# tooHotSpot/FGN

Measured on AMD Instinct MI355X. Metric: query-imgs/sec (3-way 3-shot, 800x1333 FGN simple_test), higher is better.
Workload: dtype f32; 1 GPU; cfg3: COCO2VOC 3-way 3-shot, query 3x800x1333, supports 9x3x256^2, ResNet-50-C4, R<=300 proposals, D<=100 detections, 1 episode(s) per GPU per step; h2d_in_step=True, gt_mask_rle_in_step=True, world_size_seen=1, phase_lock=rpn, caller_streams=2, support_cache=False, hip_graph=True, winograd_3x3=F(4x4,3x3)

## Files before the change

fgn_amd/csrc/conv_igemm.hip:

```cpp
#include "common.h"
#include <cstdlib>

struct ConvParams {
    const float* x = nullptr;
    const float* w = nullptr;
    float* y = nullptr;
    const float* scale = nullptr;
    const float* shift = nullptr;
    const float* residual = nullptr;
    const float* in_scale = nullptr;
    const int32_t* n_img_dev = nullptr;
    int n_img = 0, H = 1, W = 1, Cin = 0, Ho = 1, Wo = 1, Cout = 0, KH = 1, KW = 1, stride = 1, pad = 0;
    int a_img_div = 1;
    int relu = 0;
    int K = 0;
    int n_tiles_n = 0;
    int band_nt = 0, band_mt = 0;
    float* ws = nullptr;
    int splits = 1, kt_per_split = 0;
#ifdef FGN_EXPERIMENTS
    int32_t* tickets = nullptr;
    int32_t* sched = nullptr;
    int sk_U = 0, sk_dp = 0;
#endif
// ... 1160 lines not shown
        p.x = xs[i]; p.w = w_packed; p.y = ys[i]; p.scale = scale; p.shift = shift;
        p.n_img = ns[i]; p.H = Hs[i]; p.W = Ws[i]; p.Cin = Cin; p.Cout = Cout; p.KH = KH; p.KW = KW;
        p.stride = stride; p.pad = pad; p.relu = relu;
        p.Ho = g.Ho; p.Wo = g.Wo; p.K = g.K; p.x_bytes = g.x_bytes; p.w_bytes = g.w_bytes;
        p.kt_per_split = p.K / BK;
        p.n_tiles_n = cdiv(Cout, 64);
        const int m_tiles = cdiv((int)g.M, 64);
        set_band(p, 64, m_tiles, 64ll * p.K * 4);
        tiles[i] = (m_tiles * p.n_tiles_n + 7) / 8 * 8;
    }
    constexpr int NST = CONV_DMA_STAGES;
    const size_t dlds = std::max((size_t)NST * (64 + 64) * BK, (size_t)64 * (64 + 4)) * sizeof(float);
    const dim3 grid(tiles[0] + tiles[1]), wg(256);
    return Cin != 4 ? launch_kernel<conv_igemm_dma_pair_kernel<64, 64, 32, 32, NST, 4, 0>>(grid, wg, dlds, stream, ps[0], ps[1], tiles[0])
                    : launch_kernel<conv_igemm_dma_pair_kernel<64, 64, 32, 32, NST, 4, 2>>(grid, wg, dlds, stream, ps[0], ps[1], tiles[0]);
}

static int x3_pick_bm(long long M, int Cout, int K, int grp_rows, int grp_valid, int bm) {
    if (bm == 64 || bm == 128) return (grp_rows && grp_rows % bm) ? 0 : bm;
    if (grp_rows && grp_rows % 64) return 0;
    const int nt = cdiv(Cout, X3_BN);
    if (Cout * 10 < nt * X3_BN * 7) return 0;
    if (((M + 63) / 64) * nt < 192) return 0;
    const long long groups = grp_rows ? M / grp_rows : 1;
    const long long valid = grp_rows ? std::min<long long>(grp_valid > 0 ? grp_valid : grp_rows, grp_rows) : M;
    const long long rows64 = (valid + 63) / 64 * 64, rows128 = (valid + 127) / 128 * 128;
    if (K >= 256 && (!grp_rows || grp_rows % 128 == 0) && rows128 * 100 <= rows64 * 108 && groups * (rows128 / 128) * nt >= 400)
        return 128;
    return 64;
}

template <int WMW, int RB, int NT, int NST, bool SH16>
static int launch_x3_cfg(ConvParams& p, int M_max, hipStream_t stream) {
    constexpr int BM = 32 * RB * WMW;
    const int m_tiles = cdiv(M_max, BM);
    set_band(p, BM, m_tiles, (long long)X3_BN * p.K * 6);
    const int tiles = m_tiles * p.n_tiles_n;
    static unsigned long long ok = 0ull;
    hipError_t attr = fgn_allow_full_lds(reinterpret_cast<const void*>(conv_pw_x3_kernel<WMW, RB, NT, NST, SH16>), &ok);
    if (attr != hipSuccess) return (int)attr;
    const size_t lds = (size_t)NST * (BM * 128 + X3_B_STAGE);
    const int per_cu = (int)(160 * 1024 / lds);
    const int grid = std::min(256 * per_cu, (tiles + 7) / 8 * 8);
    p.stamp = fgn_next_stamp_record();
    FGN_LAUNCH_TIMED((conv_pw_x3_kernel<WMW, RB, NT, NST, SH16>), dim3(grid), dim3(128 * WMW), lds, stream, p, tiles);
    FGN_LAUNCH_CHECK();
    return FGN_OK;
}

static int launch_x3(const ConvParams& p0, int M_max, int bm, int nterms, hipStream_t stream) {
    ConvParams p = p0;
    if (!p.w3 || p.npad3 % X3_BN || p.npad3 < p.Cout || (p.Cout & 3) || p.K % BK || p.K < 2 * BK || p.splits != 1) return FGN_ERR_SHAPE;
    p.n_tiles_n = cdiv(p.Cout, X3_BN);
#ifdef FGN_EXPERIMENTS
    if (bm >= 2000) {
        const int b = bm - 2000;
        if (x3_pick_bm(M_max, p.Cout, p.K, p.grp_rows, p.grp_valid, b == 129 ? 128 : b) == 0) return FGN_ERR_SHAPE;
        if (b == 129) return nterms == 9 ? launch_x3_cfg<4, 1, 9, 3, false>(p, M_max, stream) : launch_x3_cfg<4, 1, 6, 3, false>(p, M_max, stream);
        if (b == 128) return launch_x3_cfg<2, 2, 6, 2, false>(p, M_max, stream);
        if (b == 64) return nterms == 9 ? launch_x3_cfg<2, 1, 9, 2, false>(p, M_max, stream) : launch_x3_cfg<2, 1, 6, 2, false>(p, M_max, stream);
        return FGN_ERR_SHAPE;
    }
#endif
    if (bm != 0 && bm != 64 && bm != 128) return FGN_ERR_SHAPE;
    const int BM = x3_pick_bm(M_max, p.Cout, p.K, p.grp_rows, p.grp_valid, bm);
    if (BM == 0) return FGN_ERR_SHAPE;
    if (nterms == 9) return BM == 64 ? launch_x3_cfg<2, 1, 9, 2, true>(p, M_max, stream) : FGN_ERR_SHAPE;
    return BM == 128 ? launch_x3_cfg<2, 2, 6, 2, true>(p, M_max, stream) : launch_x3_cfg<2, 1, 6, 2, true>(p, M_max, stream);
}

extern "C" size_t fgn_x3_image_bytes(int K, int npad, int n_groups) { return (size_t)n_groups * K * npad * 6; }
extern "C" int fgn_x3_row_tile(long long M, int Cout, int K, int grp_rows, int grp_valid) {
    return x3_pick_bm(M, Cout, K, grp_rows, grp_valid, 0);
}

#if defined(X3_PHASES) || defined(H2_PHASES)
static unsigned long long* g_x3_ph = nullptr;
extern "C" int fgn_x3_phases(unsigned long long* host16) {
    if (!g_x3_ph) return FGN_ERR_ARG;
    if (hipDeviceSynchronize() != hipSuccess) return FGN_ERR_ARG;
    if (hipMemcpy(host16, g_x3_ph, 128, hipMemcpyDeviceToHost) != hipSuccess) return FGN_ERR_ARG;
    return hipMemset(g_x3_ph, 0, 128) == hipSuccess ? FGN_OK : FGN_ERR_ARG;
}
#endif

static int h2_pick(long long M, int Cout, int K, int grp_rows, int grp_valid, int bm) {
    if (bm == 264) return (grp_rows && grp_rows % 128) ? 0 : 264;
    if (bm != 0) return x3_pick_bm(M, Cout, K, grp_rows, grp_valid, bm);
    if (Cout <= 64) {
        if (grp_rows && grp_rows % 128) return 0;
        if (Cout < 48 || (M + 127) / 128 < 256) return 0;
        return 264;
    }
    const int bm_x3 = x3_pick_bm(M, Cout, K, grp_rows, grp_valid, 0);
    return (bm_x3 == 128 && !grp_rows) ? 64 : bm_x3;
}

template <int WMW, int WNW, int RB, int NST, bool IM2COL, int KG = 1>
static int launch_h2_cfg(ConvParams& p, const H2Im2col& q2, int M_max, hipStream_t stream) {
    constexpr int BM = 32 * RB * WMW, BN = 64 * WNW;
    const int m_tiles = cdiv(M_max, BM);
    p.n_tiles_n = cdiv(p.Cout, BN);
    set_band(p, BM, m_tiles, (long long)BN * p.K * 4);
    const int tiles = m_tiles * p.n_tiles_n;
    static unsigned long long ok = 0ull;
    hipError_t attr = fgn_allow_full_lds(reinterpret_cast<const void*>(conv_pw_h2_kernel<WMW, WNW, RB, NST, IM2COL, KG>), &ok);
    if (attr != hipSuccess) return (int)attr;
    const size_t lds = (size_t)KG * NST * (BM * 128 + 2 * BN * 64);
    const int per_cu = std::min(3, (int)(160 * 1024 / lds));
    const int grid = std::min(256 * per_cu, (tiles + 7) / 8 * 8);
    p.stamp = fgn_next_stamp_record();
    FGN_LAUNCH_TIMED((conv_pw_h2_kernel<WMW, WNW, RB, NST, IM2COL, KG>), dim3(grid), dim3(64 * WMW * WNW * KG), lds, stream, p, q2, tiles);
    FGN_LAUNCH_CHECK();
    return FGN_OK;
}

extern "C" size_t fgn_h2_image_bytes(int K, int npad, int n_groups) { return (size_t)n_groups * npad * ((size_t)K * 4 + 4); }
extern "C" int fgn_h2_row_tile(long long M, int Cout, int K, int grp_rows, int grp_valid) {
    return h2_pick(M, Cout, K, grp_rows, grp_valid, 0);
}

constexpr int H2_KG_MIN_KTILES = 8;
constexpr int H2_BM_KG2 = 1064;
extern "C" int fgn_h2_k_groups(long long M, int Cout, int K, int grp_rows, int grp_valid) {
    if (h2_pick(M, Cout, K, grp_rows, grp_valid, 0) != 64 || grp_rows != 0 || K % BK) return 1;
    const int kt = K / BK;
    if ((kt & 1) || kt < H2_KG_MIN_KTILES) return 1;
    return cdiv(M, 64) * (long long)cdiv(Cout, H2_BN) <= 256 ? 2 : 1;
}

static int launch_h2(const ConvParams& p0, int M_max, int n_groups, int bm, hipStream_t stream, const H2Im2col* im = nullptr) {
    ConvParams p = p0;
    if (!p.w3 || p.npad3 % H2_BN || p.npad3 < p.Cout || (p.Cout & 3) || p.K % BK || p.K < 2 * BK || p.splits != 1) return FGN_ERR_SHAPE;
    const size_t img = (size_t)n_groups * p.K * p.npad3 * 4;
    p.w3_bytes = (unsigned)img;
    p.w_inv = reinterpret_cast<const float*>(static_cast<const char*>(p.w3) + img);
    H2Im2col none;
    none.y1 = nullptr; none.x_off0 = none.x_off1 = 0u; none.M0 = none.M1 = 0; none.H1 = none.W1 = none.Ho1 = none.Wo1 = 1; none.cin_shift = 0;
    if (bm != 0 && bm != 64 && bm != 128 && bm != 264 && bm != H2_BM_KG2) return FGN_ERR_SHAPE;
    if (bm == H2_BM_KG2 && ((p.K / BK) % 2 || p.K / BK < 4)) return FGN_ERR_SHAPE;
    const int cfg = h2_pick(M_max, p.Cout, p.K, p.grp_rows, p.grp_valid, bm == H2_BM_KG2 ? 64 : bm);
    if (cfg == 0) return FGN_ERR_SHAPE;
    const int kgroups = bm == H2_BM_KG2 ? 2 : (bm == 0 ? fgn_h2_k_groups(M_max, p.Cout, p.K, p.grp_rows, p.grp_valid) : 1);
    if (kgroups == 2)
        return im ? launch_h2_cfg<2, 2, 1, 2, true, 2>(p, *im, M_max, stream) : launch_h2_cfg<2, 2, 1, 2, false, 2>(p, none, M_max, stream);
    if (im) {
        if (cfg == 264) return launch_h2_cfg<4, 1, 1, 2, true>(p, *im, M_max, stream);
        return cfg == 128 ? launch_h2_cfg<2, 2, 2, 2, true>(p, *im, M_max, stream) : launch_h2_cfg<2, 2, 1, 2, true>(p, *im, M_max, stream);
    }
    if (cfg == 264) return launch_h2_cfg<4, 1, 1, 2, false>(p, none, M_max, stream);
    return cfg == 128 ? launch_h2_cfg<2, 2, 2, 2, false>(p, none, M_max, stream) : launch_h2_cfg<2, 2, 1, 2, false>(p, none, M_max, stream);
}

extern "C" int fgn_conv2d_pair_h2_bm_nhwc_f32(const float* x0, int n_img0, int H0, int W0, const float* x1, int n_img1, int H1,
                                              int W1, const void* w_h2, float* y0, float* y1, const float* scale,
                                              const float* shift, int Cin, int Cout, int cout_pad, int KH, int KW, int stride,
                                              int pad, int relu, int bm, hipStream_t stream) {
    if (!x0 || !w_h2 || !y0 || (x1 && !y1)) return FGN_ERR_ARG;
    if (n_img0 <= 0 || (x1 && n_img1 <= 0)) return FGN_ERR_SHAPE;
    const int ct = Cin / BK;
    if (Cin % BK || (ct & (ct - 1)) || KH != KW || (KW != 1 && KW != 3) || stride < 1 || pad < 0 || (Cout & 3) ||
        cout_pad % H2_BN || cout_pad < Cout || H0 <= 0 || W0 <= 0)
        return FGN_ERR_SHAPE;
    const int Ho0 = (H0 + 2 * pad - KH) / stride + 1, Wo0 = (W0 + 2 * pad - KW) / stride + 1;
    const int Ho1 = x1 ? (H1 + 2 * pad - KH) / stride + 1 : 1, Wo1 = x1 ? (W1 + 2 * pad - KW) / stride + 1 : 1;
    if (Ho0 <= 0 || Wo0 <= 0 || Ho1 <= 0 || Wo1 <= 0) return FGN_ERR_SHAPE;
// ... 71 lines not shown
}

extern "C" int fgn_conv1x1_h2_nhwc_f32(const float* x, const void* w_h2, float* y, const float* scale, const float* shift,
                                       const float* residual, const int32_t* n_img_dev, int n_img, int H, int W, int Cin,
                                       int Cout, int cout_pad, int relu, hipStream_t stream) {
    ConvParams p;
    const int rc = describe_conv1x1(p, MATH_H2, x, w_h2, y, scale, shift, residual, n_img_dev, n_img, H, W, Cin, Cout, cout_pad, relu);
    if (rc != FGN_DESCRIBED) return rc;
    return launch_h2(p, n_img * H * W, 1, 0, stream);
}

static int describe_dual(ConvParams& p, const GemmMath& m, const float* x, const float* x2, const int32_t* x2_rows,
                         int x2_total_rows, const void* w, float* y, const float* shift, int rows, int Cin1, int Cin2,
                         int Cout, int cout_pad, int relu) {
    if (!x || !x2 || !w || !y) return FGN_ERR_ARG;
    if (rows <= 0) return FGN_OK;
    if (Cin1 % BK || Cin2 % BK || Cin1 <= 0 || Cin2 <= 0 || (Cout & 3) || cout_pad % m.bn || cout_pad < Cout) return FGN_ERR_SHAPE;
    if ((!x2_rows && x2_total_rows != rows) || x2_total_rows < 1) return FGN_ERR_ARG;
    const long long K = (long long)Cin1 + Cin2;
    const long long xb = (long long)rows * Cin1 * 4, x2b = (long long)x2_total_rows * Cin2 * 4;
    const long long wb = gemm_weight_bytes(m, K, cout_pad, 1);
    if (xb >= 0x7fffff00ll || x2b >= 0x7fffff00ll || wb >= 0x7fffff00ll || (long long)rows * Cout >= (1ll << 31)) return FGN_ERR_SHAPE;
    p.x = x; p.y = y; p.shift = shift;
    p.x2 = x2; p.x2_bytes = (unsigned)x2b; p.kt1 = Cin1 / BK; p.cin2 = Cin2; p.x2_rows = x2_rows;
    p.n_img = rows; p.Cin = Cin1; p.Cout = Cout; p.relu = relu; p.K = (int)K;
    p.kt_per_split = (int)K / BK; p.x_bytes = (unsigned)xb;
    gemm_set_weights(p, m, w, wb, cout_pad);
    return FGN_DESCRIBED;
}

extern "C" int fgn_conv1x1_dual_nhwc_f32(const float* x, const float* x2, const int32_t* x2_rows, int x2_total_rows,
                                         const float* w_packed, float* y, const float* shift, int rows, int Cin1, int Cin2,
                                         int Cout, int cout_pad, int relu, hipStream_t stream) {
    ConvParams p;
    const int rc = describe_dual(p, MATH_F32, x, x2, x2_rows, x2_total_rows, w_packed, y, shift, rows, Cin1, Cin2, Cout, cout_pad, relu);
    if (rc != FGN_DESCRIBED) return rc;
    p.n_tiles_n = cdiv(Cout, 64);
    const int m_tiles = cdiv(rows, 64);
    set_band(p, 64, m_tiles, 64ll * p.K * 4);
    return launch_persist(p, m_tiles * p.n_tiles_n, stream);
}

extern "C" int fgn_conv1x1_dual_x3_nhwc_f32(const float* x, const float* x2, const int32_t* x2_rows, int x2_total_rows,
                                            const void* w_x3, float* y, const float* shift, int rows, int Cin1, int Cin2,
                                            int Cout, int cout_pad, int relu, hipStream_t stream) {
    ConvParams p;
    const int rc = describe_dual(p, MATH_X3, x, x2, x2_rows, x2_total_rows, w_x3, y, shift, rows, Cin1, Cin2, Cout, cout_pad, relu);
    if (rc != FGN_DESCRIBED) return rc;
    return launch_x3(p, rows, 0, 6, stream);
}

extern "C" int fgn_conv1x1_dual_h2_nhwc_f32(const float* x, const float* x2, const int32_t* x2_rows, int x2_total_rows,
                                            const void* w_h2, float* y, const float* shift, int rows, int Cin1, int Cin2,
                                            int Cout, int cout_pad, int relu, hipStream_t stream) {
    ConvParams p;
    const int rc = describe_dual(p, MATH_H2, x, x2, x2_rows, x2_total_rows, w_h2, y, shift, rows, Cin1, Cin2, Cout, cout_pad, relu);
    if (rc != FGN_DESCRIBED) return rc;
    return launch_h2(p, rows, 1, 0, stream);
}

static int describe_gemm(ConvParams& p, const GemmMath& m, const float* x, const void* w, float* y, const float* shift,
                         const float* residual, int rows, int K, int Cout, int npad, int relu, int grp_rows, int grp_valid,
                         int n_groups) {
    if (!x || !w || !y) return FGN_ERR_ARG;
    if (rows <= 0) return FGN_OK;
    if (K % BK || K <= 0 || (Cout & 3) || npad % m.bn || npad < Cout || n_groups < 1) return FGN_ERR_SHAPE;
    if (n_groups > 1 && (grp_rows <= 0 || (long long)n_groups * grp_rows != rows || grp_valid > grp_rows)) return FGN_ERR_SHAPE;
    const long long xb = (long long)rows * K * 4, wb = gemm_weight_bytes(m, K, npad, n_groups);
    if (xb >= 0x7fffff00ll || wb >= 0x7fffff00ll || (long long)rows * Cout >= (1ll << 31)) return FGN_ERR_SHAPE;
    p.x = x; p.y = y; p.shift = shift; p.residual = residual;
    p.n_img = rows; p.Cin = K; p.Cout = Cout; p.relu = relu; p.K = K; p.kt_per_split = K / BK; p.x_bytes = (unsigned)xb;
    p.grp_rows = n_groups > 1 ? grp_rows : 0; p.grp_valid = grp_valid;
    gemm_set_weights(p, m, w, wb, npad);
    return FGN_DESCRIBED;
}

extern "C" int fgn_gemm_x3_f32(const float* x, const void* w3, float* y, const float* shift, const float* residual,
                               int rows, int K, int Cout, int npad, int relu, int grp_rows, int grp_valid, int n_groups,
                               int bm, int nterms, hipStream_t stream) {
    ConvParams p;
    const int rc = describe_gemm(p, MATH_X3, x, w3, y, shift, residual, rows, K, Cout, npad, relu, grp_rows, grp_valid, n_groups);
    if (rc != FGN_DESCRIBED) return rc;
#ifdef X3_PHASES
    if (!g_x3_ph && (hipMalloc(&g_x3_ph, 128) != hipSuccess || hipMemset(g_x3_ph, 0, 128) != hipSuccess)) return FGN_ERR_ARG;
    p.ws = reinterpret_cast<float*>(g_x3_ph);
#endif
    return launch_x3(p, rows, bm, nterms, stream);
}

extern "C" int fgn_gemm_h2_f32(const float* x, const void* w_h2, float* y, const float* shift, const float* residual,
                               int rows, int K, int Cout, int npad, int relu, int grp_rows, int grp_valid, int n_groups,
                               int bm, hipStream_t stream) {
    ConvParams p;
    const int rc = describe_gemm(p, MATH_H2, x, w_h2, y, shift, residual, rows, K, Cout, npad, relu, grp_rows, grp_valid, n_groups);
    if (rc != FGN_DESCRIBED) return rc;
#ifdef H2_PHASES
    if (!g_x3_ph && (hipMalloc(&g_x3_ph, 128) != hipSuccess || hipMemset(g_x3_ph, 0, 128) != hipSuccess)) return FGN_ERR_ARG;
    p.ws = reinterpret_cast<float*>(g_x3_ph);
#endif
    return launch_h2(p, rows, n_groups, bm, stream);
}

extern "C" int fgn_winograd_t_pad(int tiles_total) { return (tiles_total + 127) / 128 * 128; }

static int describe_winograd_gemm(ConvParams& p, const GemmMath& m, const float* V, const void* U, float* Mo,
                                  const int32_t* n_img_dev, int n_img, int tiles_per_img, int t_pad, int Cin, int Cout,
                                  int cout_pad, int n_groups) {
    if (!V || !U || !Mo) return FGN_ERR_ARG;
    if (n_img <= 0) return FGN_OK;
    if (Cin % BK != 0 || (m.deep && Cin < 2 * BK) || Cout % 4 != 0 || cout_pad % m.bn != 0 || cout_pad < Cout || t_pad % 64 != 0 ||
        (n_groups != 16 && n_groups != 36) || (long long)n_img * tiles_per_img > t_pad)
        return FGN_ERR_SHAPE;
    const long long rows = (long long)n_groups * t_pad;
    const long long xb = rows * Cin * 4, wb = gemm_weight_bytes(m, Cin, cout_pad, n_groups);
    if (xb >= 0x7fffff00ll || wb >= 0x7fffff00ll || rows * Cout >= (1ll << 31)) return FGN_ERR_SHAPE;
    p.x = V; p.y = Mo;
    p.n_img = (int)rows; p.Cin = Cin; p.Cout = Cout; p.K = Cin; p.kt_per_split = Cin / BK; p.x_bytes = (unsigned)xb;
    p.grp_rows = t_pad; p.grp_valid = n_img * tiles_per_img; p.grp_items = n_img;
    p.grp_rows_per_item = tiles_per_img; p.grp_count_dev = n_img_dev;
    gemm_set_weights(p, m, U, wb, cout_pad);
    if (!m.image_bytes) p.grp_w_stride = cout_pad * Cin;
    return FGN_DESCRIBED;
}

extern "C" int fgn_winograd_gemm_f32(const float* V, const float* U, float* Mo, const int32_t* n_img_dev, int n_img,
                                     int tiles_per_img, int t_pad, int Cin, int Cout, int cout_pad, int n_groups,
                                     hipStream_t stream) {
    ConvParams p;
    const int rc = describe_winograd_gemm(p, MATH_F32, V, U, Mo, n_img_dev, n_img, tiles_per_img, t_pad, Cin, Cout, cout_pad, n_groups);
    if (rc != FGN_DESCRIBED) return rc;
#ifdef FGN_EXPERIMENTS
    {
        int rc2 = FGN_OK;
        if (fgn_exp_pointwise(p, p.n_img, 4, true, t_pad, stream, &rc2)) return rc2;
    }
#endif
    return launch_cfg<64, 64, 32, 32, 4>(p, p.n_img, pointwise_mode(4, p.n_img, Cout, 1), stream);
}

extern "C" int fgn_winograd_gemm_x3_f32(const float* V, const void* U_x3, float* Mo, const int32_t* n_img_dev, int n_img,
                                        int tiles_per_img, int t_pad, int Cin, int Cout, int cout_pad, int n_groups,
                                        hipStream_t stream) {
    ConvParams p;
    const int rc = describe_winograd_gemm(p, MATH_X3, V, U_x3, Mo, n_img_dev, n_img, tiles_per_img, t_pad, Cin, Cout, cout_pad, n_groups);
    if (rc != FGN_DESCRIBED) return rc;
    return launch_x3(p, p.n_img, 0, 6, stream);
}

extern "C" int fgn_winograd_gemm_h2_f32(const float* V, const void* U_h2, float* Mo, const int32_t* n_img_dev, int n_img,
                                        int tiles_per_img, int t_pad, int Cin, int Cout, int cout_pad, int n_groups,
                                        hipStream_t stream) {
    ConvParams p;
    const int rc = describe_winograd_gemm(p, MATH_H2, V, U_h2, Mo, n_img_dev, n_img, tiles_per_img, t_pad, Cin, Cout, cout_pad, n_groups);
    if (rc != FGN_DESCRIBED) return rc;
    return launch_h2(p, p.n_img, n_groups, 0, stream);
}
```

fgn_amd/csrc/conv_pw_h2.h:

```cpp
#pragma once

typedef _Float16 f16x8_t __attribute__((ext_vector_type(8)));

struct H2Frag { f16x8_t hi, lo; };

__device__ __forceinline__ void h2_split4(const float x0, const float x1, const float x2, const float x3, const float s,
                                          unsigned& h01, unsigned& h23, unsigned& l01, unsigned& l23) {
    asm("v_fma_mixlo_f16 %0, %4, %8, 0\n\t"
        "v_fma_mixlo_f16 %1, %6, %8, 0\n\t"
        "v_fma_mixhi_f16 %0, %5, %8, 0\n\t"
        "v_fma_mixhi_f16 %1, %7, %8, 0\n\t"
        "v_fma_mixlo_f16 %2, %4, %8, -%0 op_sel:[0,0,0] op_sel_hi:[0,0,1]\n\t"
        "v_fma_mixlo_f16 %3, %6, %8, -%1 op_sel:[0,0,0] op_sel_hi:[0,0,1]\n\t"
        "v_fma_mixhi_f16 %2, %5, %8, -%0 op_sel:[0,0,1] op_sel_hi:[0,0,1]\n\t"
        "v_fma_mixhi_f16 %3, %7, %8, -%1 op_sel:[0,0,1] op_sel_hi:[0,0,1]\n\t"
        "s_nop 1"
        : "=&v"(h01), "=&v"(h23), "=&v"(l01), "=&v"(l23)
        : "v"(x0), "v"(x1), "v"(x2), "v"(x3), "s"(s));
}

__device__ __forceinline__ void h2_split4_step(const int step, const float x0, const float x1, const float x2, const float x3,
                                               const float s, unsigned& h01, unsigned& h23, unsigned& l01, unsigned& l23) {
    if (step == 0)
        asm("v_fma_mixlo_f16 %0, %2, %4, 0\n\t"
            "v_fma_mixlo_f16 %1, %3, %4, 0"
            : "=&v"(h01), "=&v"(h23) : "v"(x0), "v"(x2), "s"(s));
    else if (step == 1)
        asm("v_fma_mixhi_f16 %0, %2, %4, 0\n\t"
            "v_fma_mixhi_f16 %1, %3, %4, 0"
            : "+v"(h01), "+v"(h23) : "v"(x1), "v"(x3), "s"(s));
    else if (step == 2)
        asm("v_fma_mixlo_f16 %0, %2, %4, -%5 op_sel:[0,0,0] op_sel_hi:[0,0,1]\n\t"
            "v_fma_mixlo_f16 %1, %3, %4, -%6 op_sel:[0,0,0] op_sel_hi:[0,0,1]"
            : "=&v"(l01), "=&v"(l23) : "v"(x0), "v"(x2), "s"(s), "v"(h01), "v"(h23));
    else
        asm("v_fma_mixhi_f16 %0, %2, %4, -%5 op_sel:[0,0,1] op_sel_hi:[0,0,1]\n\t"
            "v_fma_mixhi_f16 %1, %3, %4, -%6 op_sel:[0,0,1] op_sel_hi:[0,0,1]"
            : "+v"(l01), "+v"(l23) : "v"(x1), "v"(x3), "s"(s), "v"(h01), "v"(h23));
}

__device__ __forceinline__ H2Frag h2_split(const float4& a, const float4& b, const float s) {
    unsigned h[4], l[4];
    h2_split4(a.x, a.y, a.z, a.w, s, h[0], h[1], l[0], l[1]);
    h2_split4(b.x, b.y, b.z, b.w, s, h[2], h[3], l[2], l[3]);
    H2Frag f;
    f.hi = __builtin_bit_cast(f16x8_t, make_uint4(h[0], h[1], h[2], h[3]));
    f.lo = __builtin_bit_cast(f16x8_t, make_uint4(l[0], l[1], l[2], l[3]));
    return f;
}

__device__ __forceinline__ float h2_absmax16(const float4& a, const float4& b, const float4& c, const float4& d) {
    float m;
    asm("v_max3_f32 %0, |%1|, |%2|, 0\n\t"
        "v_max3_f32 %0, |%3|, |%4|, %0\n\t"
        "v_max3_f32 %0, |%5|, |%6|, %0\n\t"
        "v_max3_f32 %0, |%7|, |%8|, %0\n\t"
        "v_max3_f32 %0, |%9|, |%10|, %0\n\t"
        "v_max3_f32 %0, |%11|, |%12|, %0\n\t"
        "v_max3_f32 %0, |%13|, |%14|, %0\n\t"
        "v_max3_f32 %0, |%15|, |%16|, %0"
        : "=&v"(m)
        : "v"(a.x), "v"(a.y), "v"(a.z), "v"(a.w), "v"(b.x), "v"(b.y), "v"(b.z), "v"(b.w),
          "v"(c.x), "v"(c.y), "v"(c.z), "v"(c.w), "v"(d.x), "v"(d.y), "v"(d.z), "v"(d.w));
    return m;
}

constexpr int H2_BN = 128;

struct H2Im2col {
    float* y1;
    unsigned x_off0, x_off1;
    int M0, M1;
    int H1, W1, Ho1, Wo1;
    int cin_shift;
};

#ifdef H2_PHASES
#define H2_T(i) do { const unsigned long long now_ = __builtin_amdgcn_s_memtime(); ph_[i] += now_ - last_; last_ = now_; } while (0)
#else
#define H2_T(i) do { } while (0)
#endif
template <int WMW, int WNW, int RB, int NST, bool IM2COL, int KG = 1>
__global__ __launch_bounds__(64 * WMW * WNW * KG, KG == 1 ? 2 : 1) void conv_pw_h2_kernel(const ConvParams p, const H2Im2col q2, const int total_tiles) {
    constexpr int BM = 32 * RB * WMW, BN = 64 * WNW, NW = WMW * WNW, NTHR_G = 64 * NW, NTHR = NTHR_G * KG;
    static_assert(KG == 1 || KG == 2, "one or two K-groups");
    constexpr int A_LD = BM / 8 / NW;
    constexpr int A_STAGE = BM * 128;
    constexpr int B_STAGE = 2 * BN * 64;
    constexpr int STAGE = A_STAGE + B_STAGE;
    constexpr int BQ = BN / 16;
    constexpr int B_LD = 2 * BQ / NW;
    static_assert(A_LD * 8 * NW == BM && B_LD * NW == 2 * BQ, "tile / wave split");
    constexpr int PER = A_LD + B_LD;
    constexpr int ROWS_PER_PASS = NTHR_G / 8;
    constexpr bool OLD_CURSOR = KG == 2 && !IM2COL;
    static_assert(NST == 2, "a ring of two stages: one K-tile in flight ahead of the one being multiplied");
    extern __shared__ __attribute__((aligned(16))) unsigned char smem_h2[];

    const int t = threadIdx.x, lane = t & 63;
    const int kg = KG == 1 ? 0 : __builtin_amdgcn_readfirstlane((t >> 6) / NW);
    const int wv = KG == 1 ? t >> 6 : (t >> 6) % NW;
    const int tg = KG == 1 ? t : t % NTHR_G;
    const int wm = wv / WNW, wn = wv % WNW;
    const int M = IM2COL ? q2.M0 + q2.M1 : (p.n_img_dev ? min(p.n_img, *p.n_img_dev) : p.n_img) * p.Ho * p.Wo;
    int grp_valid = p.grp_valid;
    if (p.grp_rows && p.grp_count_dev) grp_valid = min(grp_valid, min(p.grp_items, *p.grp_count_dev) * p.grp_rows_per_item);

    float a_s = 1.f, a_inv = 1.f;

    const int col4 = tg & 7, row0 = tg >> 3;
    const int src_c4 = col4 ^ ((row0 >> 1) & 7);
    const i32x4 x_rs = make_rsrc(p.x, p.x_bytes);
    const i32x4 w_rs = make_rsrc(p.w3, p.w3_bytes);
    const bool dual = !IM2COL && p.x2 != nullptr;
    const i32x4 x2_rs = make_rsrc(dual ? p.x2 : p.x, dual ? p.x2_bytes : p.x_bytes);
    const int KT = p.K / BK / KG;
    const unsigned kt_bytes = (unsigned)(2 * p.npad3 * 64);
    const unsigned lds_base = __builtin_amdgcn_readfirstlane((unsigned)reinterpret_cast<size_t>(smem_h2) + kg * (NST * STAGE));
    const unsigned wave_row_bytes = __builtin_amdgcn_readfirstlane(wv) * 8 * 128;
    constexpr unsigned OOB = 0x7ffffff0u;

    const int nq = total_tiles >> 3, nr = total_tiles & 7;
    auto coords = [&](int tile, int& m0, int& n0) -> bool {
        const int xcd = tile & 7, idx = tile >> 3;
        const int bid = (xcd < nr ? xcd * (nq + 1) : nr * (nq + 1) + (xcd - nr) * nq) + idx;
        int tile_m = bid / p.n_tiles_n;
        int tile_n = bid - tile_m * p.n_tiles_n;
        if (p.band_nt > 0) {
            const int per_grp = p.band_mt * p.n_tiles_n;
            const int grp = bid / per_grp;
            int r = bid - grp * per_grp;
            const int per_band = p.band_mt * p.band_nt;
            const int band = r / per_band;
            r -= band * per_band;
            const int mi = r / p.band_nt;
            tile_m = grp * p.band_mt + mi;
            tile_n = band * p.band_nt + (r - mi * p.band_nt);
        }
        m0 = tile_m * BM;
        n0 = tile_n * BN;
        if (m0 >= M) return false;
        if (p.grp_rows && m0 - (m0 / p.grp_rows) * p.grp_rows >= grp_valid) return false;
        return true;
    };
    auto next_active = [&](int tile, int& m0, int& n0) -> int {
        for (; tile < total_tiles; tile += gridDim.x)
            if (coords(tile, m0, n0)) return tile;
        return -1;
    };

    struct Offs { unsigned a[A_LD], a2[A_LD], b[B_LD]; };
    unsigned b_lds[B_LD];
#pragma unroll
    for (int i = 0; i < B_LD; ++i) {
        const int q = wv + NW * i;
        b_lds[i] = __builtin_amdgcn_readfirstlane((unsigned)(A_STAGE + (q / BQ) * (BN * 64) + (q % BQ) * 1024));
    }
    auto offsets = [&](int m0, int n0) -> Offs {
        Offs o;
        const int g_end = p.grp_rows ? (m0 / p.grp_rows) * p.grp_rows + grp_valid : M;
#pragma unroll
        for (int i = 0; i < A_LD; ++i) {
            const int m = m0 + row0 + ROWS_PER_PASS * i;
            if constexpr (IM2COL) {
                o.a[i] = 0u; o.a2[i] = 0u;
                if (m < M) {
                    const bool t1 = m >= q2.M0;
                    const int mm = t1 ? m - q2.M0 : m;
                    const int H = t1 ? q2.H1 : p.H, W = t1 ? q2.W1 : p.W, Wo = t1 ? q2.Wo1 : p.Wo;
                    const int HoWo = (t1 ? q2.Ho1 : p.Ho) * Wo;
                    const int img = mm / HoWo;
                    const int rem = mm - img * HoWo;
                    const int oy = rem / Wo;
                    const int ox = rem - oy * Wo;
                    const int iy0 = oy * p.stride - p.pad, ix0 = ox * p.stride - p.pad;
                    o.a[i] = (t1 ? q2.x_off1 : q2.x_off0) + (unsigned)((((img * H + iy0) * W + ix0) * p.Cin + src_c4 * 4) * 4);
                    unsigned tm = t1 ? 0x80000000u : 0u;
                    int tp = 0;
// ... 72 lines not shown
            const unsigned voff = ok ? o.a[i] + ((o.a2[i] >> 31) ? c_off1 : c_off0) : OOB;
            lds_dma16_s(x_rs, dst, voff, 0u);
        } else {
            const bool second = c_ko >= ko1;
            i32x4 rs;
            rs[0] = second ? x2_rs[0] : x_rs[0]; rs[1] = second ? x2_rs[1] : x_rs[1];
            rs[2] = second ? x2_rs[2] : x_rs[2]; rs[3] = x_rs[3];
            lds_dma16_s(rs, dst, second ? o.a2[i] : o.a[i], second ? c_ko - ko1 : c_ko);
        }
    };

    auto issue_step = [&](const Offs& o, const int step, const unsigned wr) {
        const int kt = step * KG + kg;
        const unsigned st = lds_base + wr;
        const unsigned sa = st + wave_row_bytes;
        const unsigned ko = (unsigned)(kt * BK * 4);
        if (dual && kt >= p.kt1) {
            const unsigned ko2 = (unsigned)((kt - p.kt1) * BK * 4);
#pragma unroll
            for (int i = 0; i < A_LD; ++i) lds_dma16_s(x2_rs, sa + i * ROWS_PER_PASS * 128, o.a2[i], ko2);
        } else {
#pragma unroll
            for (int i = 0; i < A_LD; ++i) lds_dma16_s(x_rs, sa + i * ROWS_PER_PASS * 128, o.a[i], ko);
        }
        const unsigned kb = (unsigned)kt * kt_bytes;
#pragma unroll
        for (int i = 0; i < B_LD; ++i) lds_dma16_s(w_rs, st + b_lds[i], o.b[i], kb);
    };

    const int r16 = lane & 15, g4 = lane >> 4;
    const int a16_row = wm * 32 * RB + r16;
    const unsigned a16_sw = (unsigned)((a16_row >> 1) & 7);
    const unsigned a16_rd0 = (unsigned)(a16_row * 128) + ((((unsigned)g4) ^ a16_sw) << 4);
    const unsigned a16_rd1 = (unsigned)(a16_row * 128) + ((((unsigned)(g4 + 4)) ^ a16_sw) << 4);
    const int n16 = wn * 64 + r16;
    const unsigned tau16 = (0x1230u >> (4 * ((n16 >> 2) & 3))) & 3u;
    const unsigned b16_rd = (unsigned)(A_STAGE + n16 * 64) + ((((unsigned)g4) ^ tau16) << 4);

    if (p.stamp && t == 0 && blockIdx.x == 0) atomicExch(p.stamp, __builtin_amdgcn_s_memrealtime());
    auto leave = [&]() {
        if (!p.stamp || t != 0) return;
        const unsigned shard = blockIdx.x & 7u;
        const unsigned long long in_shard = (gridDim.x - shard + 7u) / 8u;
        unsigned long long* const sc = p.stamp + 8 * (1 + shard);
        if (atomicAdd(sc, 1ull) != in_shard - 1) return;
        atomicExch(sc, 0ull);
        const unsigned long long shards = gridDim.x < 8u ? gridDim.x : 8u;
        if (atomicAdd(p.stamp + 2, 1ull) != shards - 1) return;
        const unsigned long long d = __builtin_amdgcn_s_memrealtime() - atomicExch(p.stamp, 0ull);
        atomicExch(p.stamp + 2, 0ull);
        atomicAdd(p.stamp + 1, d);
        atomicAdd(p.stamp + 3, 1ull);
        atomicMin(p.stamp + 4, d);
        atomicMax(p.stamp + 5, d);
    };

    int m0, n0, nm0 = 0, nn0 = 0;
    int tile = next_active(blockIdx.x, m0, n0);
    if (tile < 0) { leave(); return; }
    Offs cur = offsets(m0, n0);
    int ntile = next_active(tile + gridDim.x, nm0, nn0);
    auto following = [&]() -> Offs { return ntile >= 0 ? offsets(nm0, nn0) : cur; };
    Offs nxt = following();
    int ic_kt = 0;
    bool ic_next = false;
    auto issue_one = [&](const unsigned wr) {
        if (!ic_next) {
            issue_step(cur, ic_kt, wr);
            if (++ic_kt == KT) { ic_next = true; ic_kt = 0; }
        } else {
            if (ntile < 0 || ic_kt >= KT) return;
            issue_step(nxt, ic_kt, wr);
            ++ic_kt;
        }
    };
    if constexpr (OLD_CURSOR) {
        issue_one(0u);
    } else {
        seek(0);
#pragma unroll
        for (int i = 0; i < PER; ++i) piece(cur, 0u, i);
        advance();
    }
    unsigned rd = 0u;
#ifdef H2_PHASES
    unsigned long long ph_[7] = {0, 0, 0, 0, 0, 0, 0}, last_ = __builtin_amdgcn_s_memtime();
    const unsigned long long begin_ = last_;
#endif

    while (true) {
        f32x4 acc[2 * RB][4];
#pragma unroll
        for (int i = 0; i < 2 * RB; ++i)
#pragma unroll
            for (int j = 0; j < 4; ++j) acc[i][j] = f32x4{0.f, 0.f, 0.f, 0.f};
        bool have_s = false;
        float a_lim = 0.f;
        a_s = 1.f; a_inv = 1.f;
        auto k_tile = [&](auto&& requests) {
            H2_T(5);
            x3_wait_vm<0>();
            asm volatile("s_waitcnt lgkmcnt(0)" ::: "memory");
            __builtin_amdgcn_s_barrier();
            asm volatile("" ::: "memory");
            H2_T(0);
            const unsigned wr = rd ^ (unsigned)STAGE;
            requests(wr);
            asm volatile("" ::: "memory");
            H2_T(1);
            const unsigned char* const S = smem_h2 + (KG == 1 ? 0 : kg * (NST * STAGE)) + rd;
            float4 alo[2 * RB], ahi[2 * RB];
            f16x8_t bq[4][2];
#pragma unroll
            for (int i = 0; i < 2 * RB; ++i) {
                alo[i] = *reinterpret_cast<const float4*>(S + a16_rd0 + i * (16 * 128));
                ahi[i] = *reinterpret_cast<const float4*>(S + a16_rd1 + i * (16 * 128));
            }
#pragma unroll
            for (int j = 0; j < 4; ++j)
#pragma unroll
                for (int q = 0; q < 2; ++q)
                    bq[j][q] = *reinterpret_cast<const f16x8_t*>(S + b16_rd + j * (16 * 64) + q * (BN * 64));
            __builtin_amdgcn_sched_barrier(0);
#ifdef H2_PHASES
            asm volatile("s_waitcnt lgkmcnt(0)" ::: "memory");
            H2_T(2);
#endif
            auto adapt = [&]() {
                auto fin = [](const float v) { const float a = fabsf(v); return a < __builtin_inff() ? a : 0.f; };
                float m = 0.f;
#pragma unroll
                for (int i = 0; i < 2 * RB; ++i) {
                    m = fmaxf(m, fmaxf(fmaxf(fin(alo[i].x), fin(alo[i].y)), fmaxf(fin(alo[i].z), fin(alo[i].w))));
                    m = fmaxf(m, fmaxf(fmaxf(fin(ahi[i].x), fin(ahi[i].y)), fmaxf(fin(ahi[i].z), fin(ahi[i].w))));
                }
#pragma unroll
                for (int o = 32; o > 0; o >>= 1) m = fmaxf(m, __shfl_xor(m, o));
                const unsigned mb = __builtin_amdgcn_readfirstlane(__float_as_uint(m));
                const int e = (int)((mb >> 23) & 0xffu);
                if (e < 27) return;
                if (have_s && __uint_as_float(mb) <= a_lim) return;
                const float ns = __uint_as_float((unsigned)(267 - e) << 23);
                const float ratio = ns * a_inv;
                if (have_s) {
#pragma unroll
                    for (int i = 0; i < 2 * RB; ++i)
#pragma unroll
                        for (int j = 0; j < 4; ++j) acc[i][j] *= ratio;
                }
                a_s = ns;
                a_inv = __uint_as_float((unsigned)(e - 13) << 23);
                a_lim = 65504.f * a_inv;
                have_s = true;
            };
            {
                float big = h2_absmax16(alo[0], ahi[0], alo[1], ahi[1]);
                if constexpr (RB == 2) big = fmaxf(big, h2_absmax16(alo[2], ahi[2], alo[3], ahi[3]));
                if (__builtin_expect(__builtin_amdgcn_ballot_w64(!(big <= a_lim)) != 0ull, 0)) adapt();
            }
            if constexpr (RB == 2 || OLD_CURSOR) {
#pragma unroll
                for (int i = 0; i < 2 * RB; ++i) {
                    const H2Frag a = h2_split(alo[i], ahi[i], a_s);
#ifdef H2_PHASES
                    if (i == 0) { asm volatile("s_nop 0" ::"v"(a.hi), "v"(a.lo)); H2_T(3); }
#endif
#pragma unroll
                    for (int j = 0; j < 4; ++j) {
                        f32x4 c = acc[i][j];
                        c = __builtin_amdgcn_mfma_f32_16x16x32_f16(a.lo, bq[j][0], c, 0, 0, 0);
                        c = __builtin_amdgcn_mfma_f32_16x16x32_f16(a.hi, bq[j][1], c, 0, 0, 0);
                        c = __builtin_amdgcn_mfma_f32_16x16x32_f16(a.hi, bq[j][0], c, 0, 0, 0);
                        acc[i][j] = c;
                    }
                }
            } else {
                unsigned fh[2][4], fl[2][4];
                h2_split4(alo[0].x, alo[0].y, alo[0].z, alo[0].w, a_s, fh[0][0], fh[0][1], fl[0][0], fl[0][1]);
                h2_split4(ahi[0].x, ahi[0].y, ahi[0].z, ahi[0].w, a_s, fh[0][2], fh[0][3], fl[0][2], fl[0][3]);
#ifdef H2_PHASES
                asm volatile("s_nop 0" ::"v"(fh[0][0]), "v"(fl[0][3]));
                H2_T(3);
#endif
#pragma unroll
                for (int i = 0; i < 2 * RB; ++i) {
                    const int u = i & 1, v = u ^ 1;
                    const f16x8_t a_hi = __builtin_bit_cast(f16x8_t, make_uint4(fh[u][0], fh[u][1], fh[u][2], fh[u][3]));
                    const f16x8_t a_lo = __builtin_bit_cast(f16x8_t, make_uint4(fl[u][0], fl[u][1], fl[u][2], fl[u][3]));
                    const int n = i + 1 < 2 * RB ? i + 1 : i;
#pragma unroll
                    for (int j = 0; j < 4; ++j) {
                        f32x4 c = acc[i][j];
#pragma unroll
                        for (int m = 0; m < 3; ++m) {
                            c = __builtin_amdgcn_mfma_f32_16x16x32_f16(m == 0 ? a_lo : a_hi, bq[j][m == 1 ? 1 : 0], c, 0, 0, 0);
                            if (m < 2 && i + 1 < 2 * RB) {
                                const int sn = 2 * j + m, half = sn >> 2;
                                const float4& x = half == 0 ? alo[n] : ahi[n];
                                h2_split4_step(sn & 3, x.x, x.y, x.z, x.w, a_s, fh[v][2 * half], fh[v][2 * half + 1],
                                               fl[v][2 * half], fl[v][2 * half + 1]);
                            }
                            __builtin_amdgcn_sched_barrier(0);
                        }
                        acc[i][j] = c;
                    }
                }
            }
#ifdef H2_PHASES
            asm volatile("s_nop 0" ::"v"(acc[0][0][0]), "v"(acc[2 * RB - 1][3][3]));
            H2_T(4);
            ++ph_[6];
#endif
            if constexpr (!OLD_CURSOR) advance();
            rd = wr;
        };
        auto request = [&](const Offs& o, const unsigned wr) {
#pragma unroll
            for (int k = 0; k < PER; ++k) piece(o, wr, k);
        };
        if constexpr (OLD_CURSOR) {
            for (int kt = 0; kt < KT; ++kt) k_tile([&](const unsigned wr) { issue_one(wr); });
        } else {
            for (int kt = 0; kt < KT - 1; ++kt) k_tile([&](const unsigned wr) { request(cur, wr); });
            seek(0);
            k_tile([&](const unsigned wr) { if (ntile >= 0) request(nxt, wr); });
        }
        float* const cbase = reinterpret_cast<float*>(smem_h2 + (rd ^ (unsigned)STAGE));
        const int em0 = m0, en0 = n0;
        const float* const winv = p.w_inv + (p.grp_rows ? (size_t)(em0 / p.grp_rows) * p.npad3 : 0);
        constexpr int PR = 32 * RB;
#pragma unroll
        for (int pass = 0; pass < WMW; ++pass) {
            __syncthreads();
            if (wm == pass && kg == 0) {
#pragma unroll
                for (int i = 0; i < 2 * RB; ++i)
#pragma unroll
                    for (int j = 0; j < 4; ++j) {
                        float* cw = cbase + (16 * i + 4 * g4) * BN + wn * 64 + 16 * j + r16;
#pragma unroll
                        for (int r = 0; r < 4; ++r) cw[r * BN] = acc[i][j][r] * a_inv;
                    }
            }
            __syncthreads();
            if constexpr (KG == 2) {
                if (wm == pass && kg == 1) {
#pragma unroll
                    for (int i = 0; i < 2 * RB; ++i)
#pragma unroll
                        for (int j = 0; j < 4; ++j) {
                            float* cw = cbase + (16 * i + 4 * g4) * BN + wn * 64 + 16 * j + r16;
#pragma unroll
                            for (int r = 0; r < 4; ++r) cw[r * BN] += acc[i][j][r] * a_inv;
                        }
                }
                __syncthreads();
            }
            constexpr int C4 = BN / 4, RPP = NTHR / C4, NPASS = PR / RPP, SW = NPASS < 4 ? NPASS : 4;
            static_assert(NPASS % SW == 0, "row sweeps in groups of SW");
            const int c4 = t % C4, rr = t / C4;
            const int n = en0 + c4 * 4;
            if (n < p.Cout) {
                float4 sc = make_float4(1.f, 1.f, 1.f, 1.f), sh = make_float4(0.f, 0.f, 0.f, 0.f);
                if (p.scale) sc = *reinterpret_cast<const float4*>(p.scale + n);
                if (p.shift) sh = *reinterpret_cast<const float4*>(p.shift + n);
                const float4 iv = *reinterpret_cast<const float4*>(winv + n);
#pragma unroll
                for (int k0 = 0; k0 < NPASS; k0 += SW) {
                    float4 res[SW];
#pragma unroll
                    for (int k = 0; k < SW; ++k) {
                        const int m = em0 + PR * pass + rr + RPP * (k0 + k);
                        res[k] = make_float4(0.f, 0.f, 0.f, 0.f);
                        if (p.residual && m < M) res[k] = *reinterpret_cast<const float4*>(p.residual + (size_t)m * p.Cout + n);
                    }
#pragma unroll
                    for (int k = 0; k < SW; ++k) {
                        const int row = rr + RPP * (k0 + k);
                        const int m = em0 + PR * pass + row;
                        if (m >= M) continue;
                        float4 v = *reinterpret_cast<const float4*>(cbase + row * BN + c4 * 4);
                        v.x *= iv.x; v.y *= iv.y; v.z *= iv.z; v.w *= iv.w;
                        v.x = v.x * sc.x + sh.x; v.y = v.y * sc.y + sh.y; v.z = v.z * sc.z + sh.z; v.w = v.w * sc.w + sh.w;
                        v.x += res[k].x; v.y += res[k].y; v.z += res[k].z; v.w += res[k].w;
                        if (p.relu) {
                            v.x = fmaxf(v.x, 0.f); v.y = fmaxf(v.y, 0.f); v.z = fmaxf(v.z, 0.f); v.w = fmaxf(v.w, 0.f);
                        }
                        float* const yrow = (IM2COL && m >= q2.M0) ? q2.y1 + (size_t)(m - q2.M0) * p.Cout : p.y + (size_t)m * p.Cout;
                        *reinterpret_cast<float4*>(yrow + n) = v;
                    }
                }
            }
        }
        if (ntile < 0) break;
        tile = ntile; m0 = nm0; n0 = nn0;
        cur = nxt;
        if constexpr (OLD_CURSOR) {
            ic_next = ic_kt >= KT;
            if (ic_next) ic_kt = 0;
        }
        ntile = next_active(tile + gridDim.x, nm0, nn0);
        nxt = following();
    }
    asm volatile("s_waitcnt vmcnt(0)" ::: "memory");
#ifdef H2_PHASES
    if (p.ws && lane == 0 && wv == 0 && kg == 0 && blockIdx.x < 2) {
        unsigned long long* o = reinterpret_cast<unsigned long long*>(p.ws) + 8 * blockIdx.x;
        for (int i = 0; i < 7; ++i) o[i] = ph_[i];
        o[7] = __builtin_amdgcn_s_memtime() - begin_;
    }
#endif
    leave();
}
```

Before: 329.0 img/s.

## Write h2 GEMM epilogue per wave through private LDS blocks without block barriers

```diff
diff --git a/fgn_amd/csrc/conv_igemm.hip b/fgn_amd/csrc/conv_igemm.hip
--- a/fgn_amd/csrc/conv_igemm.hip
+++ b/fgn_amd/csrc/conv_igemm.hip
@@ -1266,6 +1266,12 @@
     if (hipMemcpy(host16, g_x3_ph, 128, hipMemcpyDeviceToHost) != hipSuccess) return FGN_ERR_ARG;
     return hipMemset(g_x3_ph, 0, 128) == hipSuccess ? FGN_OK : FGN_ERR_ARG;
 }
+extern "C" int fgn_h2_epilogue_phases(unsigned long long* host16) {
+    if (!g_x3_ph) return FGN_ERR_ARG;
+    if (hipDeviceSynchronize() != hipSuccess) return FGN_ERR_ARG;
+    if (hipMemcpy(host16, g_x3_ph + 16, 128, hipMemcpyDeviceToHost) != hipSuccess) return FGN_ERR_ARG;
+    return hipMemset(g_x3_ph + 16, 0, 128) == hipSuccess ? FGN_OK : FGN_ERR_ARG;
+}
 #endif
 
 static int h2_pick(long long M, int Cout, int K, int grp_rows, int grp_valid, int bm) {
@@ -1503,7 +1509,7 @@
     const int rc = describe_gemm(p, MATH_X3, x, w3, y, shift, residual, rows, K, Cout, npad, relu, grp_rows, grp_valid, n_groups);
     if (rc != FGN_DESCRIBED) return rc;
 #ifdef X3_PHASES
-    if (!g_x3_ph && (hipMalloc(&g_x3_ph, 128) != hipSuccess || hipMemset(g_x3_ph, 0, 128) != hipSuccess)) return FGN_ERR_ARG;
+    if (!g_x3_ph && (hipMalloc(&g_x3_ph, 256) != hipSuccess || hipMemset(g_x3_ph, 0, 256) != hipSuccess)) return FGN_ERR_ARG;
     p.ws = reinterpret_cast<float*>(g_x3_ph);
 #endif
     return launch_x3(p, rows, bm, nterms, stream);
@@ -1516,7 +1522,7 @@
     const int rc = describe_gemm(p, MATH_H2, x, w_h2, y, shift, residual, rows, K, Cout, npad, relu, grp_rows, grp_valid, n_groups);
     if (rc != FGN_DESCRIBED) return rc;
 #ifdef H2_PHASES
-    if (!g_x3_ph && (hipMalloc(&g_x3_ph, 128) != hipSuccess || hipMemset(g_x3_ph, 0, 128) != hipSuccess)) return FGN_ERR_ARG;
+    if (!g_x3_ph && (hipMalloc(&g_x3_ph, 256) != hipSuccess || hipMemset(g_x3_ph, 0, 256) != hipSuccess)) return FGN_ERR_ARG;
     p.ws = reinterpret_cast<float*>(g_x3_ph);
 #endif
     return launch_h2(p, rows, n_groups, bm, stream);
diff --git a/fgn_amd/csrc/conv_pw_h2.h b/fgn_amd/csrc/conv_pw_h2.h
--- a/fgn_amd/csrc/conv_pw_h2.h
+++ b/fgn_amd/csrc/conv_pw_h2.h
@@ -80,6 +80,8 @@
 #else
 #define H2_T(i) do { } while (0)
 #endif
+struct H2Yes { static constexpr bool value = true; };
+struct H2No { static constexpr bool value = false; };
 template <int WMW, int WNW, int RB, int NST, bool IM2COL, int KG = 1>
 __global__ __launch_bounds__(64 * WMW * WNW * KG, KG == 1 ? 2 : 1) void conv_pw_h2_kernel(const ConvParams p, const H2Im2col q2, const int total_tiles) {
     constexpr int BM = 32 * RB * WMW, BN = 64 * WNW, NW = WMW * WNW, NTHR_G = 64 * NW, NTHR = NTHR_G * KG;
@@ -94,6 +96,18 @@
     constexpr int PER = A_LD + B_LD;
     constexpr int ROWS_PER_PASS = NTHR_G / 8;
     constexpr bool OLD_CURSOR = KG == 2 && !IM2COL;
+#ifdef H2_EPILOGUE_PASSES
+    constexpr bool WPE = false;
+#else
+    constexpr bool WPE = KG == 1;
+#endif
+#ifdef H2_PHASES
+    constexpr bool PEEL = true;
+#else
+    constexpr bool PEEL = WPE;
+#endif
+    constexpr int C_LD = 68;
+    static_assert(!WPE || NW * 16 * C_LD * 4 <= STAGE, "a 16-row block per wave fits the free stage");
     static_assert(NST == 2, "a ring of two stages: one K-tile in flight ahead of the one being multiplied");
     extern __shared__ __attribute__((aligned(16))) unsigned char smem_h2[];
 
@@ -332,9 +346,11 @@
         for (int i = 0; i < PER; ++i) piece(cur, 0u, i);
         advance();
     }
+    if constexpr (WPE) x3_wait_vm<0>();
     unsigned rd = 0u;
 #ifdef H2_PHASES
-    unsigned long long ph_[7] = {0, 0, 0, 0, 0, 0, 0}, last_ = __builtin_amdgcn_s_memtime();
+    bool walked = false;
+    unsigned long long ph_[14] = {0, 0, 0, 0, 0, 0, 0, 0, 0, 0, 0, 0, 0, 0}, last_ = __builtin_amdgcn_s_memtime();
     const unsigned long long begin_ = last_;
 #endif
 
@@ -347,9 +363,22 @@
         bool have_s = false;
         float a_lim = 0.f;
         a_s = 1.f; a_inv = 1.f;
-        auto k_tile = [&](auto&& requests) {
-            H2_T(5);
-            x3_wait_vm<0>();
+        float4 res_e[4];
+        auto residual_rows = [&](const int i) {
+            const int n = n0 + wn * 64 + r16 * 4;
+#pragma unroll
+            for (int k = 0; k < 4; ++k) {
+                const int m = m0 + wm * (32 * RB) + 16 * i + g4 + 4 * k;
+                res_e[k] = make_float4(0.f, 0.f, 0.f, 0.f);
+                if (p.residual && m < M && n < p.Cout) res_e[k] = *reinterpret_cast<const float4*>(p.residual + (size_t)m * p.Cout + n);
+            }
+        };
+        auto k_tile = [&](auto&& requests, auto first) {
+            if constexpr (decltype(first)::value) H2_T(12); else H2_T(5);
+            if constexpr (!(WPE && decltype(first)::value)) x3_wait_vm<0>();
+#ifdef H2_PHASES
+            if (decltype(first)::value && walked) H2_T(7);
+#endif
             asm volatile("s_waitcnt lgkmcnt(0)" ::: "memory");
             __builtin_amdgcn_s_barrier();
             asm volatile("" ::: "memory");
@@ -469,19 +498,73 @@
             for (int k = 0; k < PER; ++k) piece(o, wr, k);
         };
         if constexpr (OLD_CURSOR) {
-            for (int kt = 0; kt < KT; ++kt) k_tile([&](const unsigned wr) { issue_one(wr); });
+            for (int kt = 0; kt < KT; ++kt) k_tile([&](const unsigned wr) { issue_one(wr); }, H2No{});
         } else {
-            for (int kt = 0; kt < KT - 1; ++kt) k_tile([&](const unsigned wr) { request(cur, wr); });
+            if constexpr (PEEL) k_tile([&](const unsigned wr) { request(cur, wr); }, H2Yes{});
+            for (int kt = PEEL ? 1 : 0; kt < KT - 1; ++kt) k_tile([&](const unsigned wr) { request(cur, wr); }, H2No{});
             seek(0);
-            k_tile([&](const unsigned wr) { if (ntile >= 0) request(nxt, wr); });
+            k_tile([&](const unsigned wr) { if (ntile >= 0) request(nxt, wr); }, H2No{});
         }
         float* const cbase = reinterpret_cast<float*>(smem_h2 + (rd ^ (unsigned)STAGE));
         const int em0 = m0, en0 = n0;
         const float* const winv = p.w_inv + (p.grp_rows ? (size_t)(em0 / p.grp_rows) * p.npad3 : 0);
+        if constexpr (WPE) {
+            residual_rows(0);
+            asm volatile("s_waitcnt lgkmcnt(0)" ::: "memory");
+            __builtin_amdgcn_s_barrier();
+            asm volatile("" ::: "memory");
+            H2_T(8);
+            float* const cw0 = cbase + wv * (16 * C_LD);
+            const int n = en0 + wn * 64 + r16 * 4;
+            const bool n_in = n < p.Cout;
+            float4 sc = make_float4(1.f, 1.f, 1.f, 1.f), sh = make_float4(0.f, 0.f, 0.f, 0.f), iv = make_float4(0.f, 0.f, 0.f, 0.f);
+            if (n_in) {
+                if (p.scale) sc = *reinterpret_cast<const float4*>(p.scale + n);
+                if (p.shift) sh = *reinterpret_cast<const float4*>(p.shift + n);
+                iv = *reinterpret_cast<const float4*>(winv + n);
+            }
+#pragma unroll
+            for (int i = 0; i < 2 * RB; ++i) {
+#pragma unroll
+                for (int j = 0; j < 4; ++j)
+#pragma unroll
+                    for (int r = 0; r < 4; ++r) cw0[(4 * g4 + r) * C_LD + 16 * j + r16] = acc[i][j][r] * a_inv;
+                asm volatile("s_waitcnt lgkmcnt(0)" ::: "memory");
+                H2_T(9);
+                if (i == 0) {
+                    x3_wait_vm<0>();
+                    H2_T(10);
+                }
+                float4 res[4];
+#pragma unroll
+                for (int k = 0; k < 4; ++k) res[k] = res_e[k];
+                if (i + 1 < 2 * RB) residual_rows(i + 1);
+#pragma unroll
+                for (int k = 0; k < 4; ++k) {
+                    const int row = g4 + 4 * k;
+                    const int m = em0 + wm * (32 * RB) + 16 * i + row;
+                    if (m >= M || !n_in) continue;
+                    float4 v = *reinterpret_cast<const float4*>(cw0 + row * C_LD + r16 * 4);
+                    v.x *= iv.x; v.y *= iv.y; v.z *= iv.z; v.w *= iv.w;
+                    v.x = v.x * sc.x + sh.x; v.y = v.y * sc.y + sh.y; v.z = v.z * sc.z + sh.z; v.w = v.w * sc.w + sh.w;
+                    v.x += res[k].x; v.y += res[k].y; v.z += res[k].z; v.w += res[k].w;
+                    if (p.relu) {
+                        v.x = fmaxf(v.x, 0.f); v.y = fmaxf(v.y, 0.f); v.z = fmaxf(v.z, 0.f); v.w = fmaxf(v.w, 0.f);
+                    }
+                    float* const yrow = (IM2COL && m >= q2.M0) ? q2.y1 + (size_t)(m - q2.M0) * p.Cout : p.y + (size_t)m * p.Cout;
+                    *reinterpret_cast<float4*>(yrow + n) = v;
+                }
+                asm volatile("" ::: "memory");
+                H2_T(11);
+            }
+        }
         constexpr int PR = 32 * RB;
 #pragma unroll
-        for (int pass = 0; pass < WMW; ++pass) {
+        for (int pass = 0; pass < (WPE ? 0 : WMW); ++pass) {
             __syncthreads();
+#ifdef H2_PHASES
+            if (pass == 0) H2_T(8);
+#endif
             if (wm == pass && kg == 0) {
 #pragma unroll
                 for (int i = 0; i < 2 * RB; ++i)
@@ -506,6 +589,7 @@
                 }
                 __syncthreads();
             }
+            H2_T(9);
             constexpr int C4 = BN / 4, RPP = NTHR / C4, NPASS = PR / RPP, SW = NPASS < 4 ? NPASS : 4;
             static_assert(NPASS % SW == 0, "row sweeps in groups of SW");
             const int c4 = t % C4, rr = t / C4;
@@ -524,6 +608,10 @@
                         res[k] = make_float4(0.f, 0.f, 0.f, 0.f);
                         if (p.residual && m < M) res[k] = *reinterpret_cast<const float4*>(p.residual + (size_t)m * p.Cout + n);
                     }
+#ifdef H2_PHASES
+                    x3_wait_vm<0>();
+                    H2_T(10);
+#endif
 #pragma unroll
                     for (int k = 0; k < SW; ++k) {
                         const int row = rr + RPP * (k0 + k);
@@ -539,9 +627,17 @@
                         float* const yrow = (IM2COL && m >= q2.M0) ? q2.y1 + (size_t)(m - q2.M0) * p.Cout : p.y + (size_t)m * p.Cout;
                         *reinterpret_cast<float4*>(yrow + n) = v;
                     }
-                }
-            }
-        }
+#ifdef H2_PHASES
+                    asm volatile("" ::: "memory");
+                    H2_T(11);
+#endif
+                }
+            }
+        }
+#ifdef H2_PHASES
+        ++ph_[13];
+        walked = true;
+#endif
         if (ntile < 0) break;
         tile = ntile; m0 = nm0; n0 = nn0;
         cur = nxt;
@@ -558,6 +654,7 @@
         unsigned long long* o = reinterpret_cast<unsigned long long*>(p.ws) + 8 * blockIdx.x;
         for (int i = 0; i < 7; ++i) o[i] = ph_[i];
         o[7] = __builtin_amdgcn_s_memtime() - begin_;
+        for (int i = 7; i < 14; ++i) o[16 + i - 7] = ph_[i];
     }
 #endif
     leave();
```

Result: faster. 332.9 img/s (median of 6 runs) (+1.2%).
